# torchipeppo/prb-project-bearing-only-slam

Measured on AMD Instinct MI355X. Metric: GN iterations/sec + observations/sec (J+H build) at 1/2/4/8 GPUs vs CPU, higher is better.
Workload: dtype f32

## Files before the change

include/bos_host.h:

```cpp
#ifndef BOS_HOST_H_
#define BOS_HOST_H_

#include "bos.h"

#ifdef __cplusplus
extern "C" {
#endif

typedef struct bos_dataset bos_dataset;

int bos_dataset_load_g2o(const char* path, int triangulate, int verbose, bos_dataset** out);
int bos_dataset_synthetic(int32_t num_poses, int32_t num_landmarks, int32_t bearings_per_pose, uint64_t seed,
                          bos_dataset** out);
int bos_dataset_problem(const bos_dataset* ds, bos_problem* view);
const int32_t* bos_dataset_pose_ids(const bos_dataset* ds);
const int32_t* bos_dataset_landmark_ids(const bos_dataset* ds);
int32_t bos_dataset_fixed_pose_id(const bos_dataset* ds);
float bos_dataset_bound(const bos_dataset* ds);
int bos_dataset_ground_truth(const bos_dataset* ds, const double** pose_xyt, const double** landmark_xy);
int bos_dataset_write_g2o(const bos_dataset* ds, const char* path, const double* pose_xyt, const double* landmark_xy,
                          int with_landmarks);
void bos_dataset_free(bos_dataset* ds);

double bos_normalized_angle_f64(double a);
// ... 93 lines not shown

int bos_time_linearize(struct bos_solver* s, int32_t n, int32_t flush_caches, double* ms_per_build);
int bos_time_triangulate(struct bos_solver* s, int32_t n, double* ms_per_call);
int bos_time_steps(struct bos_solver* s, int32_t n, double* ms_per_step);

int bos_marginals_timing(const struct bos_solver* s, double ms[4], int64_t* sigma_bytes);
int bos_edge_covariances_timing(const struct bos_solver* s, double ms[5], int64_t* edge_bytes);
int bos_pair_covariances_timing(const struct bos_solver* s, double ms[6], int64_t* bytes);
int bos_node_covariances_timing(const struct bos_solver* s, double ms[7], int64_t* bytes);
int bos_associate_bearings_timing(const struct bos_solver* s, double ms[8], int64_t* bytes);
int bos_debug_set_associate_chunk(struct bos_solver* s, int64_t max_bearings);
int bos_match_timing(const struct bos_solver* s, double ms[8], int64_t* bytes);
int bos_debug_set_match_chunk(struct bos_solver* s, int64_t max_rows);
int bos_debug_set_pair_batch(struct bos_solver* s, int64_t max_distinct_nodes);
int bos_time_cost(struct bos_solver* s, int32_t n, double* ms_per_pass);

int bos_time_facade_steps(const bos_problem* problem, const bos_options* options, int32_t n, double* ms_per_step,
                          double* ms_state_read, double* ms_per_step_capi, int64_t* mismatches);
int bos_debug_facade_selftest(const bos_problem* problem, const bos_options* options, int32_t n, int64_t* mismatches);

void bos_debug_set_g2o_parser(int32_t line_by_line);
int bos_debug_inject_stall(struct bos_solver* s);
int bos_debug_set_step_graph(struct bos_solver* s, int32_t enable);
int bos_debug_solver_stamps(struct bos_solver* s, int64_t capacity, uint64_t* stamps, int32_t* meta);

enum {
    BOS_ROUTE_NONE = -1,
    BOS_ROUTE_F_REG16 = 0,
    BOS_ROUTE_F_REG16_SIDE = 1,
    BOS_ROUTE_F_PAN48 = 2,
    BOS_ROUTE_F_PAN64 = 3,
    BOS_ROUTE_F_PAN64_SIDE = 4,
    BOS_ROUTE_F_BLK = 5,
    BOS_ROUTE_F_BLK_SIDE2 = 6,
    BOS_ROUTE_F_MIXB_BLK = 7,
    BOS_ROUTE_F_MIXB_WAVE = 8,
    BOS_ROUTE_F_LEVEL = 9,
    BOS_ROUTE_F_FLOW = 10,
    BOS_ROUTE_F_FOLDED = 11,
    BOS_ROUTE_F_COUNT = 12
};
enum {
    BOS_ROUTE_B_FLOW = 0,
    BOS_ROUTE_B_WAVE = 1,
    BOS_ROUTE_B_LEVEL = 2,
    BOS_ROUTE_B_FOLD = 3,
// ... 22 lines not shown
```

prb-project-bearing-only-slam_amd/bos.py:

```python
from __future__ import annotations

import ctypes
import os
from typing import Optional

import numpy as np

_HERE = os.path.dirname(os.path.abspath(__file__))
LIB_PATH = os.path.join(_HERE, "lib", "libbos.so")
ALLOW_MISSING_SYMBOLS = False

BOS_OK = 0
BOS_FP64 = 64
BOS_FP32 = 32
BOS_SOLVER_SUPERNODAL = 0
BOS_SOLVER_DENSE_CHOL = 1
BOS_SOLVER_ROCSOLVER_RF = 2
BOS_SOLVER_SCHUR = 3
BOS_SOLVER_SPARSE_CHOL = BOS_SOLVER_SCHUR
BOS_PARTITION_SUBTREE = 0
BOS_PARTITION_OBSERVATIONS = 1
ABI_VERSION = 3

EXPORTED_SYMBOLS = [
    "bos_default_options", "bos_last_error", "bos_abi_version", "bos_device_count", "bos_device_peer_access",
    "bos_nccl_unique_id",
    "bos_create", "bos_destroy", "bos_set_kernel_threshold", "bos_set_damping_factor", "bos_step", "bos_step_n",
    "bos_linearize", "bos_linearize_async", "bos_synchronize", "bos_system_info_get", "bos_export_system",
    "bos_get_state", "bos_set_state", "bos_get_last_dx",
    "bos_dataset_load_g2o", "bos_dataset_synthetic", "bos_dataset_problem", "bos_dataset_pose_ids",
    "bos_dataset_landmark_ids", "bos_dataset_fixed_pose_id", "bos_dataset_bound", "bos_dataset_ground_truth",
    "bos_dataset_write_g2o", "bos_dataset_free", "bos_plan_inspect", "bos_plan_mf_selftest",
    "bos_debug_linearize_timeline", "bos_triangulate", "bos_triangulate_async", "bos_plan_shard_selftest",
    "bos_plan_node_owner", "bos_step_phase", "bos_exchange_size", "bos_exchange_download", "bos_exchange_upload",
    "bos_node_owner",
    "bos_debug_set_g2o_parser", "bos_debug_inject_stall", "bos_debug_set_step_graph", "bos_debug_solver_stamps",
    "bos_debug_solver_routes", "bos_debug_selinv_fronts", "bos_plan_mf_fronts",
    "bos_time_linearize", "bos_time_triangulate", "bos_time_steps", "bos_cpu_gn_create", "bos_cpu_gn_step", "bos_cpu_gn_get_state",
    "bos_cpu_gn_destroy", "bos_normalized_angle_f64", "bos_normalized_angle_f32", "bos_exchange_p2p_handle",
    "bos_exchange_p2p_connect", "bos_time_facade_steps", "bos_debug_facade_selftest", "bos_set_exchange_timeout",
    "bos_last_step_stamps", "bos_marginals", "bos_plan_mf_marginals", "bos_marginals_timing",
    "bos_lm_default_options", "bos_cost", "bos_optimize", "bos_time_cost", "bos_cpu_gn_set_kernel_threshold",
    "bos_cpu_gn_cost", "bos_cpu_gn_optimize", "bos_lm_rule_apply",
    "bos_edge_covariances", "bos_plan_mf_edge_covariances", "bos_edge_covariances_timing",
    "bos_pair_covariances", "bos_plan_mf_pair_covariances", "bos_plan_pair_paths", "bos_pair_covariances_timing",
    "bos_debug_set_pair_batch",
    "bos_node_covariances", "bos_plan_mf_node_covariances", "bos_node_covariances_timing",
    "bos_associate_bearings", "bos_plan_mf_associate_bearings", "bos_associate_bearings_timing",
    "bos_debug_set_associate_chunk", "bos_associate_tile",
    "bos_match_landmarks", "bos_match_poses", "bos_plan_mf_match_landmarks", "bos_plan_mf_match_poses",
    "bos_match_information_inverse", "bos_match_timing", "bos_debug_set_match_chunk",
]

LM_STOP_DX, LM_STOP_COST, LM_STOP_ITERATIONS, LM_STOP_LAMBDA = 1, 2, 3, 4
LM_MAX_ITERATIONS = 4096

P2P_HANDLE_BYTES = 64

_dp = ctypes.POINTER(ctypes.c_double)
_ip = ctypes.POINTER(ctypes.c_int32)
# ... 173 lines not shown
        "bos_cost": (ctypes.c_int, [vp, _dp, _dp, _ip]),
        "bos_optimize": (ctypes.c_int, [vp, ctypes.POINTER(bos_lm_options), ctypes.POINTER(bos_lm_result),
                                        ctypes.POINTER(bos_lm_iteration), ctypes.c_int32]),
        "bos_time_cost": (ctypes.c_int, [vp, ctypes.c_int32, _dp]),
        "bos_cpu_gn_set_kernel_threshold": (ctypes.c_int, [vp, ctypes.c_double]),
        "bos_cpu_gn_cost": (ctypes.c_int, [vp, _dp, _dp, _ip]),
        "bos_cpu_gn_optimize": (ctypes.c_int, [vp, ctypes.POINTER(bos_lm_options), ctypes.POINTER(bos_lm_result),
                                               ctypes.POINTER(bos_lm_iteration), ctypes.c_int32]),
        "bos_lm_rule_apply": (ctypes.c_int, [ctypes.POINTER(bos_lm_state), ctypes.POINTER(bos_lm_options), ctypes.c_double,
                                             ctypes.c_double, ctypes.c_double, ctypes.c_int32,
                                             ctypes.POINTER(bos_lm_iteration)]),
        "bos_plan_shard_selftest": (ctypes.c_int, [ctypes.POINTER(bos_problem), ctypes.POINTER(bos_options), ctypes.c_int32,
                                                   _dp, _dp, _dp]),
        "bos_plan_node_owner": (ctypes.c_int, [ctypes.POINTER(bos_problem), ctypes.POINTER(bos_options), ctypes.c_int32, _ip]),
        "bos_step_phase": (ctypes.c_int, [vp, ctypes.c_int32, ctypes.POINTER(bos_step_stats)]),
        "bos_exchange_size": (ctypes.c_int, [vp, ctypes.c_int32, ctypes.POINTER(ctypes.c_int64)]),
        "bos_exchange_download": (ctypes.c_int, [vp, ctypes.c_int32, _dp]),
        "bos_exchange_upload": (ctypes.c_int, [vp, ctypes.c_int32, _dp]),
        "bos_node_owner": (ctypes.c_int, [vp, _ip]),
        "bos_debug_set_g2o_parser": (None, [ctypes.c_int32]),
        "bos_debug_inject_stall": (ctypes.c_int, [vp]),
        "bos_debug_set_step_graph": (ctypes.c_int, [vp, ctypes.c_int32]),
        "bos_debug_solver_routes": (ctypes.c_int, [vp, ctypes.c_int64, _ip, _ip]),
        "bos_debug_selinv_fronts": (ctypes.c_int, [vp, ctypes.c_int64, _ip, _ip, _ip, _ip]),
        "bos_plan_mf_fronts": (ctypes.c_int, [ctypes.POINTER(bos_problem), ctypes.POINTER(bos_options), ctypes.c_int64, _ip, _ip]),
        "bos_debug_solver_stamps": (ctypes.c_int, [vp, ctypes.c_int64, ctypes.POINTER(ctypes.c_uint64),
                                                   ctypes.POINTER(ctypes.c_int32)]),
        "bos_time_linearize": (ctypes.c_int, [vp, ctypes.c_int32, ctypes.c_int32, _dp]),
        "bos_time_triangulate": (ctypes.c_int, [vp, ctypes.c_int32, _dp]),
        "bos_time_steps": (ctypes.c_int, [vp, ctypes.c_int32, _dp]),
        "bos_cpu_gn_create": (ctypes.c_int, [ctypes.POINTER(bos_problem), ctypes.c_int32, ctypes.c_int32,
                                             ctypes.POINTER(vp)]),
        "bos_cpu_gn_step": (ctypes.c_int, [vp, _dp]),
        "bos_cpu_gn_get_state": (ctypes.c_int, [vp, _dp, _dp]),
        "bos_cpu_gn_destroy": (None, [vp]),
        "bos_exchange_p2p_handle": (ctypes.c_int, [vp, ctypes.c_void_p]),
        "bos_exchange_p2p_connect": (ctypes.c_int, [vp, ctypes.c_void_p]),
        "bos_set_exchange_timeout": (ctypes.c_int, [vp, ctypes.c_double]),
        "bos_last_step_stamps": (ctypes.c_int, [vp, ctypes.POINTER(ctypes.c_uint64)]),
        "bos_normalized_angle_f64": (ctypes.c_double, [ctypes.c_double]),
        "bos_normalized_angle_f32": (ctypes.c_float, [ctypes.c_float]),
        "bos_time_facade_steps": (ctypes.c_int, [ctypes.POINTER(bos_problem), ctypes.POINTER(bos_options), ctypes.c_int32,
                                                 _dp, _dp, _dp, ctypes.POINTER(ctypes.c_int64)]),
        "bos_debug_facade_selftest": (ctypes.c_int, [ctypes.POINTER(bos_problem), ctypes.POINTER(bos_options),
                                                     ctypes.c_int32, ctypes.POINTER(ctypes.c_int64)]),
    }
# ... 409 lines not shown
    a, b, _ = _pair_cov_arrays(node_a, node_b, False, False, False)
    out = np.zeros((len(a), len(PAIR_PATH_COLS)), dtype=np.int32)
    opt = options(solver, schur_leaf=schur_leaf)
    _check(lib().bos_plan_pair_paths(ctypes.byref(cs), ctypes.byref(opt), len(a), _ptr(a, ctypes.c_int32),
                                     _ptr(b, ctypes.c_int32), _ptr(out, ctypes.c_int32)), "plan_pair_paths")
    return out


PLAN_FRONT_COLS = ("k", "r", "level", "parent", "children", "folded_children", "folded", "diag_records", "cross_rj",
                   "cross_jj", "cross_transposed")


def plan_mf_fronts(P: Problem, solver: int = BOS_SOLVER_SCHUR, schur_leaf: int = 0) -> np.ndarray:
    cs = P.c_struct()
    opt = options(solver, schur_leaf=schur_leaf)
    n = ctypes.c_int32(0)
    _check(lib().bos_plan_mf_fronts(ctypes.byref(cs), ctypes.byref(opt), 0, None, ctypes.byref(n)), "plan_mf_fronts")
    out = np.zeros((n.value, len(PLAN_FRONT_COLS)), dtype=np.int32)
    _check(lib().bos_plan_mf_fronts(ctypes.byref(cs), ctypes.byref(opt), out.size, _ptr(out, ctypes.c_int32),
                                    ctypes.byref(n)), "plan_mf_fronts")
    return out


def plan_shard_selftest(P: Problem, world: int, vals, rhs, solver: int = BOS_SOLVER_SCHUR):
    cs = P.c_struct()
    v = np.ascontiguousarray(vals, dtype=np.float64)
    b = np.ascontiguousarray(rhs, dtype=np.float64)
    x = np.zeros_like(b)
    opt = options(solver)
    _check(lib().bos_plan_shard_selftest(ctypes.byref(cs), ctypes.byref(opt), world, _ptr(v, ctypes.c_double),
                                         _ptr(b, ctypes.c_double), _ptr(x, ctypes.c_double)), "plan_shard_selftest")
    return x


def plan_node_owner(P: Problem, world: int, solver: int = BOS_SOLVER_SCHUR) -> np.ndarray:
    cs = P.c_struct()
    o = np.zeros(P.NP + P.NL, dtype=np.int32)
    opt = options(solver)
    _check(lib().bos_plan_node_owner(ctypes.byref(cs), ctypes.byref(opt), world, _ptr(o, ctypes.c_int32)),
           "plan_node_owner")
    return o


def lm_options(**opts) -> bos_lm_options:
    o = bos_lm_options()
    lib().bos_lm_default_options(ctypes.byref(o))
# ... 222 lines not shown
        out = np.zeros((n.value, 4), dtype=np.int32)
        _check(lib().bos_debug_solver_routes(self._h, out.size, _ptr(out, ctypes.c_int32), ctypes.byref(n)),
               "bos_debug_solver_routes")
        return out

    SELINV_CLASSES = ("wave_lds", "blk_lds_mfma", "blk_workspace")
    SELINV_COLS = ("class", "launch", "k", "r", "folded", "sigma_front", "diag_records", "cross_rj", "cross_jj",
                   "cross_transposed")

    def debug_selinv_fronts(self) -> dict:
        n = ctypes.c_int32(0)
        _check(lib().bos_debug_selinv_fronts(self._h, 0, None, ctypes.byref(n), None, None), "bos_debug_selinv_fronts")
        fronts = np.zeros((n.value, len(self.SELINV_COLS)), dtype=np.int32)
        node = np.zeros(self.P.NP + self.P.NL, dtype=np.int32)
        edge = np.zeros(len(self.P.b_z) + len(self.P.o_z), dtype=np.int32)
        _check(lib().bos_debug_selinv_fronts(self._h, fronts.size, _ptr(fronts, ctypes.c_int32), ctypes.byref(n),
                                             _ptr(node, ctypes.c_int32), _ptr(edge, ctypes.c_int32)),
               "bos_debug_selinv_fronts")
        return {"fronts": fronts, "node_front": node, "edge_front": edge}

    def debug_set_step_graph(self, enable: bool):
        _check(lib().bos_debug_set_step_graph(self._h, int(enable)), "bos_debug_set_step_graph")

    def time_linearize(self, n: int, flush_caches: bool = False) -> float:
        ms = ctypes.c_double(0)
        _check(lib().bos_time_linearize(self._h, n, int(flush_caches), ctypes.byref(ms)), "bos_time_linearize")
        return ms.value

    def time_steps(self, n: int) -> float:
        ms = ctypes.c_double(0)
        _check(lib().bos_time_steps(self._h, n, ctypes.byref(ms)), "bos_time_steps")
        return ms.value

    def time_triangulate(self, n: int) -> float:
        ms = ctypes.c_double(0)
        _check(lib().bos_time_triangulate(self._h, n, ctypes.byref(ms)), "bos_time_triangulate")
        return ms.value

    def triangulate(self):
        _check(lib().bos_triangulate(self._h), "bos_triangulate")

    def triangulate_async(self):
        _check(lib().bos_triangulate_async(self._h), "bos_triangulate_async")

    def synchronize(self):
        _check(lib().bos_synchronize(self._h), "bos_synchronize")
# ... 163 lines not shown
```

prb-project-bearing-only-slam_amd/csrc/hip/mf_backward.hpp:

```cpp
#pragma once

#include <hip/hip_runtime.h>

#include <cstdint>

#include "mf_device.hpp"
#include "mf_flow.hpp"
#include "wave_util.hpp"

namespace bos {
namespace dev {

namespace {

constexpr int kBwdRegK = 32;

template <int MODE>
__device__ __forceinline__ void backward_front(const MfArgs& a, int s, double* w, int lane, const Flow* f,
                                               const int32_t* parent) {
    constexpr bool COH = MODE == kModeFlow;
    const int k = a.k[s], r = a.r[s], m = k + r;
    const int c0 = a.col0[s];
    const int32_t* fi = a.findex + a.findex_off[s];
    double* t = w + k;
// ... 147 lines not shown
    }
    if (head) {
        const double x1 = (y1 - t1) / L11;
        t0 += L10 * x1;
        a.x[c0] = (y0 - t0) / L00;
        a.x[c0 + 1] = x1;
    }
}

__global__ __launch_bounds__(64) void mf_backward_flow(const MfArgs a, const Flow f_in, const int32_t* parent) {
    extern __shared__ __attribute__((aligned(16))) double w[];
    Flow f = f_in;
    f.epoch = *f_in.epoch_src;
    for (int it = 0; it <= f.n; ++it) {
        const int t = next_ticket(f.ticket);
        if (t >= f.n) break;
        const int s = f.order[t];
        backward_front<kModeFlow>(a, s, w, threadIdx.x, &f, parent);
        fstamp(f.stamps, s, 4);
    }
    leave_flow(f);
}

}

}
}
```

prb-project-bearing-only-slam_amd/csrc/hip/multifrontal.hip:

```cpp
#include <hip/hip_runtime.h>

#include <algorithm>
#include <cstdint>
#include <string>
#include <vector>

#include "../../../include/bos_host.h"
#include "../host/plan.hpp"
#include "device_mem.hpp"
#include "mf_backward.hpp"
#include "mf_blk.hpp"
#include "mf_device.hpp"
#include "mf_flow.hpp"
#include "mf_level.hpp"
#include "mf_wave.hpp"
#include "multifrontal.hpp"
#include "selinv.hpp"

namespace bos {
namespace dev {

constexpr int kClasses = 6;
inline int front_class(int m) { return m <= kMfWaveMaxM ? (m - 1) / 16 : m <= kBlkMaxM ? 4 : 5; }
inline int launch_class(int m) {
    const int c = front_class(m);
    return c == 1 ? 2 : c;
}

struct Prog {
    int id = 0;
// ... 47 lines not shown
    hipStream_t side = nullptr, side2 = nullptr;
    hipEvent_t ev_fork = nullptr, ev_join = nullptr, ev_join2 = nullptr;
    static constexpr int tiny16 = 256;
    Prog prog[2];
    int8_t *fid_f = nullptr, *fid_b = nullptr;
    int32_t* parent = nullptr;
    int* tickets = nullptr;
    uint32_t* epoch = nullptr;
    unsigned long long* stamps = nullptr;
    int32_t *fold_cnt = nullptr, *fold_cptr = nullptr, *fold_chunk = nullptr, *fold_rec = nullptr;
    int16_t* emap = nullptr;
    int64_t* emap_off = nullptr;
    int32_t *col0 = nullptr, *k = nullptr, *r = nullptr, *child_ptr = nullptr, *child = nullptr,
            *rmap = nullptr, *amap_ptr = nullptr, *amap_src = nullptr, *amap_dst = nullptr, *findex = nullptr,
            *info = nullptr;
    int64_t *L_off = nullptr, *U_off = nullptr, *u_off = nullptr, *scratch_off = nullptr, *rmap_off = nullptr,
            *findex_off = nullptr;
    double *L = nullptr, *U = nullptr, *u = nullptr, *scratch = nullptr;
    const float* A32 = nullptr;
    int64_t pl_lo = 0;
    unsigned long long *Ug = nullptr, *xg = nullptr;
    int64_t* ug_off = nullptr;
    int8_t* xtag = nullptr;
    SelInv* selinv = nullptr;
    std::vector<int8_t> route_f, route_b;
    std::vector<int32_t> h_child_ptr, h_child, h_fold_cnt;
    bool noted_f[2] = {false, false}, noted_b[2] = {false, false};
    void note_f(int which, int route, const int32_t* fronts, int n) {
        if (noted_f[which]) return;
        for (int i = 0; i < n; ++i) {
            const int s = fronts[i];
            route_f[s] = (int8_t)route;
            if (!h_fold_cnt.empty())
                for (int ci = h_child_ptr[s]; ci < h_child_ptr[s] + h_fold_cnt[s]; ++ci)
                    route_f[h_child[ci]] = (int8_t)BOS_ROUTE_F_FOLDED;
        }
    }
    void note_b(int which, int route, const int32_t* fronts, int n) {
        if (noted_b[which]) return;
        for (int i = 0; i < n; ++i) route_b[fronts[i]] = (int8_t)route;
    }

    MfArgs args(const Prog& P, int lev, int c, const double* A, double* x) const {
        MfArgs g;
        g.level = P.list + (P.ptr.empty() ? 0 : P.ptr[lev * kClasses + c]);
        g.count = P.ptr.empty() ? 0 : P.count(lev, c);
// ... 165 lines not shown
    auto up = [&](auto** p, const auto& v) { return mem.upload(p, v, kMfPad); };
    auto bad = [&] { err = "device allocation or upload failed (multifrontal)"; return -2; };
    if (!(up(&d->fid_f, fid_f) && up(&d->fid_b, fid_b) && up(&d->parent, F.parent))) return bad();
    {
        std::vector<int64_t> ugo(F.nsuper, -1);
        int64_t ug_size = 0, ndof = 0;
        for (int c = 0; c < F.nsuper; ++c) {
            ndof = std::max<int64_t>(ndof, (int64_t)F.col0[c] + F.k[c]);
            const int p = F.parent[c];
            if (p < 0 || fid_f[c] == 0 || fid_f[p] != fid_f[c]) continue;
            const int64_t rc2 = F.r[c];
            ugo[c] = ug_size;
            ug_size += 2 * (rc2 * (rc2 + 1) / 2 + rc2);
        }
        std::vector<int8_t> xt(F.nsuper, 0);
        for (int c = 0; c < F.nsuper; ++c)
            if (fid_b[c] != 0)
                for (int q = c; q >= 0 && !xt[q]; q = F.parent[q]) xt[q] = 1;
        if (!(up(&d->ug_off, ugo) && up(&d->xtag, xt) && mem.alloc(&d->Ug, std::max<int64_t>(ug_size, 1), true, 2 * kMfPad) &&
              mem.alloc(&d->xg, std::max<int64_t>(2 * ndof, 1), true, 2 * kMfPad)))
            return bad();
    }
    if (!(mem.alloc(&d->tickets, 2 * kMfTickets, true) && mem.upload(&d->epoch, std::vector<uint32_t>{1}))) return bad();
    {
        std::vector<int64_t> eoff(F.nsuper, 0);
        std::vector<int16_t> em;
        for (int c = 0; c < F.nsuper; ++c) {
            const int p = F.parent[c];
            if (p < 0) continue;
            const int mp = F.k[p] + F.r[p], rc = F.r[c];
            if (mp > kBlkMaxM || rc == 0) continue;
            bool folded = false;
            for (int ci = F.child_ptr[p]; ci < F.child_ptr[p] + (F.fold_cnt.empty() ? 0 : F.fold_cnt[p]); ++ci)
                folded = folded || F.child[ci] == c;
            if (folded) continue;
            eoff[c] = (int64_t)em.size();
            const int32_t* rm = F.rmap.data() + F.rmap_off[c];
            for (int j = 0; j < rc; ++j)
                for (int i = j; i < rc; ++i) {
                    const int I = rm[i], J = rm[j];
                    if (I < J || I >= mp) { err = "multifrontal: child row map not increasing"; return -1; }
                    em.push_back((int16_t)(mp <= kMfWaveMaxM ? J * mp - J * (J - 1) / 2 + (I - J) : I + J * mp));
                }
        }
        if (!(up(&d->emap, em) && up(&d->emap_off, eoff))) return bad();
    }
// ... 110 lines not shown
                     d->fid_f, P.id, d->stamps};
        const int grid = std::min(P.n_flow_factor, d->ncu * kFlowWavesFactor);
        hipLaunchKernelGGL((mf_factor_flow<F32>), dim3(grid), dim3(64), 0, s, d->args(P, 0, 0, A, x), f);
        d->note_f(which, BOS_ROUTE_F_FLOW, P.h_order_factor.data(), P.n_flow_factor);
        if ((e = hipGetLastError()) != hipSuccess) return e;
    }
    d->noted_f[which] = true;
    return hipSuccess;
}

hipError_t mf_factor(MfDevice* d, int which, const double* A, double* x, hipStream_t s) {
    return d->A32 ? mf_factor_t<true>(d, which, A, x, s) : mf_factor_t<false>(d, which, A, x, s);
}

void mf_set_fold_source(MfDevice* d, const float* A32, int64_t pl_lo) {
    d->A32 = A32;
    d->pl_lo = pl_lo;
}

hipError_t mf_solve(MfDevice* d, int which, double* x, hipStream_t s) {
    hipError_t e;
    const Prog& P = d->prog[which];
    if (P.ptr.empty()) return hipSuccess;
    if (P.flow_solve) {
        const Flow fb{P.order_bwd, P.n_flow_solve, d->tickets + 1, d->tickets + kMfTickets + 1,
                      d->epoch, 0u, d->fid_b, P.id, d->stamps ? d->stamps + 8 * (int64_t)d->nsuper : nullptr};
        const int grid = std::min(P.n_flow_solve, d->ncu * kFlowWavesBackward);
        hipLaunchKernelGGL(mf_backward_flow, dim3(grid), dim3(64), P.lds_bwd_flow, s, d->args(P, 0, 0, nullptr, x), fb,
                           (const int32_t*)d->parent);
        d->note_b(which, BOS_ROUTE_B_FLOW, P.h_order_bwd.data(), P.n_flow_solve);
        if ((e = hipGetLastError()) != hipSuccess) return e;
    }
    for (int l = std::min(P.solve_lev0, d->nlevels) - 1; l >= 0; --l) {
        int n;
        if (P.bptr[l + 1] > P.bptr[l]) {
            MfArgs g = d->args(P, l, 0, nullptr, x);
            g.level = P.blist + P.bptr[l];
            g.count = P.bptr[l + 1] - P.bptr[l];
            hipLaunchKernelGGL(mf_backward_wave, dim3(g.count), dim3(64), P.blds[l], s, g);
            d->note_b(which, BOS_ROUTE_B_WAVE, P.h_blist.data() + P.bptr[l], g.count);
        }
        if ((n = P.count(l, 4, kClasses))) {
            MfArgs g = d->args(P, l, 4, nullptr, x);
            g.count = n;
            hipLaunchKernelGGL(mf_backward_level, dim3(n), dim3(kMfBlock), P.lds_max(P.lds_bwd, l, 4, kClasses), s, g);
            d->note_b(which, BOS_ROUTE_B_LEVEL, P.hl(l, 4), n);
        }
        if ((e = hipGetLastError()) != hipSuccess) return e;
    }
    if (P.n_fold > 0) {
        MfArgs g = d->args(P, 0, 0, nullptr, x);
        g.level = P.fold_list;
        g.count = P.n_fold;
        hipLaunchKernelGGL(mf_backward_fold, dim3(((int64_t)P.n_fold * kFoldLanes + kMfBlock - 1) / kMfBlock), dim3(kMfBlock), 0, s, g);
        d->note_b(which, BOS_ROUTE_B_FOLD, P.h_fold_list.data(), P.n_fold);
        if ((e = hipGetLastError()) != hipSuccess) return e;
    }
    d->noted_b[which] = true;
    return hipSuccess;
}

int mf_debug_routes(const MfDevice* d, int8_t* factor, int8_t* backward) {
    for (int w = 0; w < 2; ++w)
        if (!d->prog[w].ptr.empty() && (!d->noted_f[w] || !d->noted_b[w])) return -1;
    std::copy(d->route_f.begin(), d->route_f.end(), factor);
    std::copy(d->route_b.begin(), d->route_b.end(), backward);
    return 0;
}

MfView mf_view(const MfDevice* d) { return MfView{d->k, d->r, d->parent, d->rmap, d->L_off, d->rmap_off, d->L}; }
SelInv** mf_selinv_slot(MfDevice* d) { return &d->selinv; }
int32_t* mf_info_ptr(const MfDevice* d) { return d->info; }
uint32_t* mf_epoch_ptr(const MfDevice* d) { return d->epoch; }
void mf_debug_set_stamps(MfDevice* d, unsigned long long* stamps) {
    d->stamps = stamps;
#ifdef BOS_MF_PIVOT_CYCLES
    unsigned long long* b = stamps ? stamps + 8 * (int64_t)d->nsuper : nullptr;
    (void)hipMemcpyToSymbol(HIP_SYMBOL(g_pivot_bwd), &b, sizeof(b));
#endif
}
int32_t* mf_tickets_ptr(const MfDevice* d) { return d->tickets; }
double* mf_update_ptr(const MfDevice* d) { return d->U; }
double* mf_uvec_ptr(const MfDevice* d) { return d->u; }

hipError_t mf_debug_skip_next_front(MfDevice* d, hipStream_t s) {
    if (d->prog[0].n_flow_factor == 0 || !d->prog[0].first_waited) return hipErrorInvalidValue;
    static const int one = 1;
    return hipMemcpyAsync(d->tickets, &one, sizeof(int), hipMemcpyHostToDevice, s);
}

// ... 3 lines not shown
```

prb-project-bearing-only-slam_amd/csrc/hip/multifrontal.hpp:

```cpp
#pragma once

#include <hip/hip_runtime.h>

#include <string>

namespace bos {
struct Multifrontal;
namespace dev {

struct MfDevice;

int mf_create(const Multifrontal& F, const int8_t* owner, int rank, MfDevice** out, std::string& err);
void mf_destroy(MfDevice* d);
hipError_t mf_factor(MfDevice* d, int program, const double* A, double* x, hipStream_t s);
void mf_set_fold_source(MfDevice* d, const float* A32, int64_t pl_lo);
hipError_t mf_solve(MfDevice* d, int program, double* x, hipStream_t s);
double* mf_update_ptr(const MfDevice* d);
double* mf_uvec_ptr(const MfDevice* d);
int32_t* mf_info_ptr(const MfDevice* d);
uint32_t* mf_epoch_ptr(const MfDevice* d);
void mf_debug_set_stamps(MfDevice* d, unsigned long long* stamps);
constexpr int32_t kMfStall = 1 << 30;
int mf_debug_routes(const MfDevice* d, int8_t* factor, int8_t* backward);
int32_t* mf_tickets_ptr(const MfDevice* d);
constexpr int kMfTickets = 3;
struct MfView {
    const int32_t *k, *r, *parent, *rmap;
    const int64_t *L_off, *rmap_off;
    const double* L;
};
MfView mf_view(const MfDevice* d);
struct SelInv;
SelInv** mf_selinv_slot(MfDevice* d);
hipError_t mf_debug_skip_next_front(MfDevice* d, hipStream_t s);

}
}
```

prb-project-bearing-only-slam_amd/csrc/hip/solver_step.hip:

```cpp
#include <algorithm>
#include <atomic>
#include <chrono>
#include <cstring>

#include "solver_handle.hpp"

using namespace bos::capi;

namespace {

template <typename T> bos::dev::LinParams<T> lin_params(const bos_solver* s) {
    bos::dev::LinParams<T> p;
    p.pc = (const T*)s->d_pc;
    p.pth = (const T*)s->d_pth;
    p.lc = (const T*)s->d_lc;
    const bos::Plan& P = s->plan;
    p.NP = s->NP;
    p.lane_pose = s->lane_identity ? nullptr : s->lane_pose;
    p.n_groups = (int)P.blk.lane_pose.size();
    p.n_lm_lanes = (int)P.blk.lm_lane_lm.size();
    p.pose_blocks = s->pose_blocks;
    p.pose_b0 = (int)s->pose_b0;
    p.n_pose_run = (int)s->n_pose_run;
    p.lm_b0 = (int)s->lm_b0;
// ... 574 lines not shown
    const bos::Multifrontal& F = s->plan.mf;
    if (nsuper) *nsuper = F.nsuper;
    if (!routes && capacity == 0 && nsuper) return BOS_OK;
    if (!routes || capacity < 4 * (int64_t)F.nsuper) return fail(BOS_ERR_INVALID, "routes: capacity 4 * supernodes");
    std::vector<int8_t> rf(F.nsuper), rb(F.nsuper);
    if (bos::dev::mf_debug_routes(s->mf, rf.data(), rb.data()))
        return fail(BOS_ERR_INVALID, "routes: no step has been enqueued on this handle yet");
    for (int x = 0; x < F.nsuper; ++x) {
        routes[4 * x] = rf[x];
        routes[4 * x + 1] = rb[x];
        routes[4 * x + 2] = F.k[x];
        routes[4 * x + 3] = F.r[x];
    }
    return BOS_OK;
}

int bos_debug_set_step_graph(bos_solver* s, int32_t enable) {
    if (!s) return fail(BOS_ERR_INVALID, "null handle");
    drop_graph(s);
    s->graph_failed = !enable;
    return BOS_OK;
}

int bos_triangulate(bos_solver* s) {
    if (!s) return fail(BOS_ERR_INVALID, "null handle");
    HIP_TRY(hipSetDevice(s->device));
    int rc = enqueue_triangulate(s);
    if (rc) return rc;
    HIP_TRY(hipStreamSynchronize(s->stream));
    s->have_dx = false;
    return BOS_OK;
}

int bos_triangulate_async(bos_solver* s) {
    if (!s) return fail(BOS_ERR_INVALID, "null handle");
    return enqueue_triangulate(s);
}

int bos_synchronize(bos_solver* s) {
    if (!s) return fail(BOS_ERR_INVALID, "null handle");
    HIP_TRY(hipStreamSynchronize(s->stream));
    return BOS_OK;
}

int bos_linearize(bos_solver* s, bos_step_stats* st) {
    if (!s) return fail(BOS_ERR_INVALID, "null handle");
// ... 141 lines not shown
```

prb-project-bearing-only-slam_amd/csrc/host/capi_host.cpp:

```cpp
#include <chrono>
#include <cstdio>
#include <cstdlib>
#include <algorithm>
#include <cmath>
#include <cstring>
#include <functional>
#include <memory>
#include <stdexcept>
#include <string>
#include <vector>

#include "../../../include/bos_host.h"
#include "associate.hpp"
#include "match.hpp"
#include "edge_cov.hpp"
#include "node_cov.hpp"
#include "pair_cov.hpp"
#include "g2o_utils.hpp"
#include "host_mf.hpp"
#include "plan.hpp"
#include "synthetic.hpp"
#include "triangulation.hpp"

#include "error.hpp"

namespace {
int hfail(int code, const std::string& m) { return bos::set_error(code, m); }
}

struct bos_dataset {
    proj02::State state;
    proj02::BearingObservationVector bearings;
    proj02::OdometryObservationVector odometry;
    int fixed_pose_id = -1;
    float bound = 0;
    std::vector<double> pose_xyt, lm_xy, b_z, o_z, o_om;
// ... 341 lines not shown
    for (int32_t x : F.fold_list) folded[x] = 1;
    std::vector<int32_t> out_ptr, out_rec;
    bos::CrossRecords cr;
    if (!bos::selinv_records(P, out_ptr, out_rec) ||
        !bos::selinv_cross_records(P, pi.Mb, pi.Mo, pi.b_pose, pi.b_lm, pi.o_src, pi.o_dst, cr))
        return hfail(BOS_ERR_UNSUPPORTED, "a node or an edge's cross block is not inside one front");
    for (int x = 0; x < F.nsuper; ++x) {
        int32_t* o = fronts + (size_t)BOS_PLAN_FRONT_COLS * x;
        o[0] = F.k[x]; o[1] = F.r[x]; o[2] = lev[x]; o[3] = F.parent[x];
        o[4] = F.child_ptr[x + 1] - F.child_ptr[x];
        o[5] = F.fold_cnt.empty() ? 0 : F.fold_cnt[x];
        o[6] = folded[x];
        o[7] = out_ptr[x + 1] - out_ptr[x];
        o[8] = o[9] = o[10] = 0;
        for (int q = cr.ptr[x]; q < cr.ptr[x + 1]; ++q) {
            const int32_t* rec = cr.rec.data() + (size_t)bos::kCrossRec * q;
            ++o[rec[0] >= F.k[x] ? 8 : 9];
            o[10] += rec[5];
        }
    }
    return BOS_OK;
}

int bos_plan_mf_selftest(const bos_problem* pb, const bos_options* options, const double* vals, const double* rhs,
                         double* x) {
    if (!pb || !vals || !rhs || !x) return hfail(BOS_ERR_INVALID, "null argument");
    bos::ProblemIndex pi;
    bos_options opt;
    int fmode = 0;
    int rc = plan_args(pb, options, pi, fmode, opt);
    if (rc) return rc;
    if (opt.solver != BOS_SOLVER_SUPERNODAL && opt.solver != BOS_SOLVER_SCHUR)
        return hfail(BOS_ERR_INVALID, "selftest needs a multifrontal solver");
    bos::Plan P;
    std::string err;
    rc = bos::build_plan(pi, 0, 1, fmode, P, err);
    if (rc) return hfail(rc, err);
    bos::HostMf M(P, vals, rhs);
    auto all = [](int) { return true; };
    M.factor(all);
    M.forward(all);
    M.backward(all);
    std::copy(M.x.begin(), M.x.end(), x);
    return BOS_OK;
}

// ... 523 lines not shown
```

Measured before the change: 87.86 billion.

## Solve top supernodal levels with one wave per root-to-leaf path

Adds a backward-solve route where each base-level front gets a single wave that walks its chain of ancestors to the root. Each wave redundantly recomputes the shared upper fronts in its own LDS copy of the solution, and it prefetches the next front's panel into registers while solving the current one. This replaces the per-level launches or ticket-based flow solve for the upper levels and so removes inter-front synchronisation and launch overhead. The cost is redundant work on shared ancestors, an extra kernel that saves the right-hand side first, and a limit on LDS and front size. The route is on by default when the plan qualifies, and it falls back when occupancy is insufficient.

```diff
diff --git a/include/bos_host.h b/include/bos_host.h
--- a/include/bos_host.h
+++ b/include/bos_host.h
@@ -139,6 +139,10 @@
 void bos_debug_set_g2o_parser(int32_t line_by_line);
 int bos_debug_inject_stall(struct bos_solver* s);
 int bos_debug_set_step_graph(struct bos_solver* s, int32_t enable);
+int bos_debug_set_backward_path(struct bos_solver* s, int32_t enable);
+int bos_debug_backward_path_info(struct bos_solver* s, int32_t* out);
+int bos_plan_backward_path(const bos_problem* problem, const bos_options* options, int32_t world, int32_t* info,
+                           int32_t* fronts, int32_t* base, int32_t* path_ptr, int32_t* path, int32_t* rows);
 int bos_debug_solver_stamps(struct bos_solver* s, int64_t capacity, uint64_t* stamps, int32_t* meta);
 
 enum {
diff --git a/prb-project-bearing-only-slam_amd/bos.py b/prb-project-bearing-only-slam_amd/bos.py
--- a/prb-project-bearing-only-slam_amd/bos.py
+++ b/prb-project-bearing-only-slam_amd/bos.py
@@ -36,6 +36,7 @@
     "bos_node_owner",
     "bos_debug_set_g2o_parser", "bos_debug_inject_stall", "bos_debug_set_step_graph", "bos_debug_solver_stamps",
     "bos_debug_solver_routes", "bos_debug_selinv_fronts", "bos_plan_mf_fronts",
+    "bos_debug_set_backward_path", "bos_debug_backward_path_info", "bos_plan_backward_path",
     "bos_time_linearize", "bos_time_triangulate", "bos_time_steps", "bos_cpu_gn_create", "bos_cpu_gn_step", "bos_cpu_gn_get_state",
     "bos_cpu_gn_destroy", "bos_normalized_angle_f64", "bos_normalized_angle_f32", "bos_exchange_p2p_handle",
     "bos_exchange_p2p_connect", "bos_time_facade_steps", "bos_debug_facade_selftest", "bos_set_exchange_timeout",
@@ -255,6 +256,10 @@
         "bos_debug_inject_stall": (ctypes.c_int, [vp]),
         "bos_debug_set_step_graph": (ctypes.c_int, [vp, ctypes.c_int32]),
         "bos_debug_solver_routes": (ctypes.c_int, [vp, ctypes.c_int64, _ip, _ip]),
+        "bos_debug_set_backward_path": (ctypes.c_int, [vp, ctypes.c_int32]),
+        "bos_debug_backward_path_info": (ctypes.c_int, [vp, _ip]),
+        "bos_plan_backward_path": (ctypes.c_int, [ctypes.POINTER(bos_problem), ctypes.POINTER(bos_options), ctypes.c_int32,
+                                                  _ip, _ip, _ip, _ip, _ip, _ip]),
         "bos_debug_selinv_fronts": (ctypes.c_int, [vp, ctypes.c_int64, _ip, _ip, _ip, _ip]),
         "bos_plan_mf_fronts": (ctypes.c_int, [ctypes.POINTER(bos_problem), ctypes.POINTER(bos_options), ctypes.c_int64, _ip, _ip]),
         "bos_debug_solver_stamps": (ctypes.c_int, [vp, ctypes.c_int64, ctypes.POINTER(ctypes.c_uint64),
@@ -710,6 +715,24 @@
     return out
 
 
+def plan_backward_path(P: Problem, solver: int = BOS_SOLVER_SCHUR, schur_leaf: int = 0, world: int = 1) -> dict:
+    cs = P.c_struct()
+    opt = options(solver, schur_leaf=schur_leaf)
+    info = np.zeros(8, dtype=np.int32)
+    ip = lambda a: _ptr(a, ctypes.c_int32)
+    _check(lib().bos_plan_backward_path(ctypes.byref(cs), ctypes.byref(opt), world, ip(info), None, None, None, None, None),
+           "plan_backward_path")
+    fronts = np.zeros((info[4], 7), dtype=np.int32)
+    base = np.zeros(max(info[1], 1), dtype=np.int32)
+    path_ptr = np.zeros(info[1] + 1, dtype=np.int32)
+    path = np.zeros(max(info[5], 1), dtype=np.int32)
+    rows = np.zeros((max(info[6], 1), 2), dtype=np.int32)
+    _check(lib().bos_plan_backward_path(ctypes.byref(cs), ctypes.byref(opt), world, ip(info), ip(fronts), ip(base),
+                                        ip(path_ptr), ip(path), ip(rows)), "plan_backward_path")
+    return {"base_level": int(info[0]), "base_fronts": int(info[1]), "longest_path": int(info[2]), "lds_bytes": int(info[3]),
+            "fronts": fronts, "base": base[:info[1]], "path_ptr": path_ptr, "path": path[:info[5]], "rows": rows[:info[6]]}
+
+
 def plan_shard_selftest(P: Problem, world: int, vals, rhs, solver: int = BOS_SOLVER_SCHUR):
     cs = P.c_struct()
     v = np.ascontiguousarray(vals, dtype=np.float64)
@@ -978,6 +1001,14 @@
     def debug_set_step_graph(self, enable: bool):
         _check(lib().bos_debug_set_step_graph(self._h, int(enable)), "bos_debug_set_step_graph")
 
+    def debug_set_backward_path(self, enable: bool):
+        _check(lib().bos_debug_set_backward_path(self._h, int(enable)), "bos_debug_set_backward_path")
+
+    def backward_path_info(self) -> dict:
+        out = np.zeros(4, dtype=np.int32)
+        _check(lib().bos_debug_backward_path_info(self._h, _ptr(out, ctypes.c_int32)), "bos_debug_backward_path_info")
+        return dict(zip(("base_level", "base_fronts", "longest_path", "lds_bytes"), (int(v) for v in out)))
+
     def time_linearize(self, n: int, flush_caches: bool = False) -> float:
         ms = ctypes.c_double(0)
         _check(lib().bos_time_linearize(self._h, n, int(flush_caches), ctypes.byref(ms)), "bos_time_linearize")
diff --git a/prb-project-bearing-only-slam_amd/csrc/hip/mf_backward.hpp b/prb-project-bearing-only-slam_amd/csrc/hip/mf_backward.hpp
--- a/prb-project-bearing-only-slam_amd/csrc/hip/mf_backward.hpp
+++ b/prb-project-bearing-only-slam_amd/csrc/hip/mf_backward.hpp
@@ -193,7 +193,145 @@
     leave_flow(f);
 }
 
-}
-
-}
-}
+struct PathArgs {
+    const int32_t *k, *r, *col0;
+    const int64_t *L_off, *findex_off;
+    const double* L;
+    double* x;
+    unsigned long long* stamps;
+    const int32_t* path_ptr;
+    const int32_t* path;
+    const int32_t* pbase;
+    const int32_t* rowpos;
+    const int32_t* stamper;
+    const double* y;
+    int nx;
+};
+
+__global__ __launch_bounds__(256) void mf_path_save_y(const int32_t* dof, int n, const double* x, double* y) {
+    const int i = blockIdx.x * 256 + threadIdx.x;
+    if (i < n) y[dof[i]] = x[dof[i]];
+}
+
+constexpr int kPathPre = 8;
+struct PathMeta {
+    int k, r, c0, pb;
+    int64_t L_off, fi_off;
+};
+struct PathPre {
+    double v[kPathPre], y;
+    int pos;
+};
+
+__device__ __forceinline__ int64_t readlane_i64(int64_t x, int l) {
+    const int lo = __builtin_amdgcn_readlane((int)(x & 0xffffffffll), l);
+    const int hi = __builtin_amdgcn_readlane((int)(x >> 32), l);
+    return ((int64_t)hi << 32) | (unsigned int)lo;
+}
+
+__device__ __forceinline__ PathMeta path_meta(const PathMeta& mine, int i) {
+    PathMeta f;
+    f.k = __builtin_amdgcn_readlane(mine.k, i);
+    f.r = __builtin_amdgcn_readlane(mine.r, i);
+    f.c0 = __builtin_amdgcn_readlane(mine.c0, i);
+    f.pb = __builtin_amdgcn_readlane(mine.pb, i);
+    f.L_off = readlane_i64(mine.L_off, i);
+    f.fi_off = readlane_i64(mine.fi_off, i);
+    return f;
+}
+
+__device__ __forceinline__ void path_prefetch(const PathArgs& p, const PathMeta& f, int lane, PathPre& o) {
+    const double* src = p.L + f.L_off;
+    const int n = (f.k + f.r) * f.k;
+#pragma unroll
+    for (int u = 0; u < kPathPre; ++u) o.v[u] = src[min(64 * u + lane, n - 1)];
+    o.y = p.y[f.c0 + min(lane, f.k - 1)];
+    o.pos = p.rowpos[f.fi_off + f.k + min(lane, max(f.r - 1, 0))];
+}
+
+template <int KR>
+__device__ __forceinline__ double path_chain_reg(const double* Lw, int k, int m, int lane, bool own, int col, double yv,
+                                                 double tj, double rjj) {
+    double lr[KR], xv = 0.0;
+#pragma unroll
+    for (int j = 0; j < KR; ++j) lr[j] = own && j < k ? Lw[j + col * m] : 0.0;
+#pragma unroll
+    for (int j = KR - 1; j >= 0; --j) {
+        if (j < k) {
+            const double xj = readlane_d((yv - tj) * rjj, j);
+            if (lane == j) xv = xj;
+            else if (lane < j) tj += lr[j] * xj;
+        }
+    }
+    return xv;
+}
+
+__global__ __launch_bounds__(64) void mf_backward_path(const PathArgs p) {
+    extern __shared__ __attribute__((aligned(16))) double w[];
+    double* const xp = w;
+    double* const Lw = w + p.nx;
+    const int lane = threadIdx.x, b = blockIdx.x;
+    const int p0 = p.path_ptr[b], n = p.path_ptr[b + 1] - p0;
+    PathMeta mine;
+    {
+        const int s = p.path[p0 + min(lane, n - 1)];
+        mine.k = p.k[s];
+        mine.r = p.r[s];
+        mine.c0 = p.col0[s];
+        mine.pb = p.pbase[s];
+        mine.L_off = p.L_off[s];
+        mine.fi_off = p.findex_off[s];
+    }
+    PathMeta f = path_meta(mine, 0);
+    PathPre pre;
+    path_prefetch(p, f, lane, pre);
+    for (int i = 0; i < n; ++i) {
+        const int k = f.k, r = f.r, m = k + r, c0 = f.c0, pb = f.pb;
+        int s = 0;
+        unsigned long long* stp = nullptr;
+        if (p.stamps) {
+            s = p.path[p0 + i];
+            stp = p.stamper[s] == b ? p.stamps : nullptr;
+        }
+        fstamp(stp, s, 0);
+#pragma unroll
+        for (int u = 0; u < kPathPre; ++u)
+            if (64 * u + lane < m * k) Lw[64 * u + lane] = pre.v[u];
+        if (m * k > 64 * kPathPre)
+            stage_lds<8, false>(Lw + 64 * kPathPre, p.L + f.L_off + 64 * kPathPre, m * k - 64 * kPathPre, lane);
+        const bool own = lane < k;
+        const int col = own ? lane : 0;
+        const double yv = own ? pre.y : 0.0;
+        const double xr = xp[lane < r ? pre.pos : 0];
+        wave_sync();
+        fstamp(stp, s, 1);
+        fstamp(stp, s, 2);
+        f = path_meta(mine, min(i + 1, n - 1));
+        path_prefetch(p, f, lane, pre);
+        const double rjj = own ? 1.0 / Lw[col + col * m] : 1.0;
+        double tj = 0.0;
+        for (int q = 0; q < r; ++q) tj += Lw[k + q + col * m] * readlane_d(xr, q);
+        double xv = 0.0;
+        if (k <= 16) xv = path_chain_reg<16>(Lw, k, m, lane, own, col, yv, tj, rjj);
+        else if (k <= kBwdRegK) xv = path_chain_reg<kBwdRegK>(Lw, k, m, lane, own, col, yv, tj, rjj);
+        else {
+            for (int j = k - 1; j >= 0; --j) {
+                const double xj = readlane_d((yv - tj) * rjj, j);
+                if (lane == j) xv = xj;
+                else if (lane < j) tj += Lw[j + col * m] * xj;
+            }
+        }
+        if (own) {
+            xp[pb + lane] = xv;
+            p.x[c0 + lane] = xv;
+        }
+        wave_sync();
+        fstamp(stp, s, 3);
+        fstamp(stp, s, 4);
+    }
+}
+
+}
+
+}
+}
diff --git a/prb-project-bearing-only-slam_amd/csrc/hip/multifrontal.hip b/prb-project-bearing-only-slam_amd/csrc/hip/multifrontal.hip
--- a/prb-project-bearing-only-slam_amd/csrc/hip/multifrontal.hip
+++ b/prb-project-bearing-only-slam_amd/csrc/hip/multifrontal.hip
@@ -6,6 +6,7 @@
 #include <vector>
 
 #include "../../../include/bos_host.h"
+#include "../host/backward_path.hpp"
 #include "../host/plan.hpp"
 #include "device_mem.hpp"
 #include "mf_backward.hpp"
@@ -99,6 +100,12 @@
     unsigned long long *Ug = nullptr, *xg = nullptr;
     int64_t* ug_off = nullptr;
     int8_t* xtag = nullptr;
+    BackwardPath bp;
+    bool path_on = true;
+    int32_t *bp_path_ptr = nullptr, *bp_path = nullptr, *bp_pbase = nullptr, *bp_rowpos = nullptr, *bp_stamper = nullptr,
+            *bp_ydof = nullptr;
+    double* bp_y = nullptr;
+    std::vector<int32_t> h_path_fronts;
     SelInv* selinv = nullptr;
     std::vector<int8_t> route_f, route_b;
     std::vector<int32_t> h_child_ptr, h_child, h_fold_cnt;
@@ -310,6 +317,30 @@
             return bad();
     }
     if (!(mem.alloc(&d->tickets, 2 * kMfTickets, true) && mem.upload(&d->epoch, std::vector<uint32_t>{1}))) return bad();
+    if (!owner) {
+        BackwardPath& bp = d->bp;
+        build_backward_path(F, bp);
+        int resident = 0;
+        if (bp.on() &&
+            (hipOccupancyMaxActiveBlocksPerMultiprocessor(&resident, mf_backward_path, 64, bp.lds_bytes) != hipSuccess ||
+             (int64_t)resident * d->ncu < (int64_t)bp.base.size())) {
+            (void)hipGetLastError();
+            bp = BackwardPath();
+        }
+        if (bp.on()) {
+            std::vector<int32_t> stamper(F.nsuper, -1);
+            for (size_t b = 0; b < bp.base.size(); ++b)
+                for (int q = bp.path_ptr[b]; q < bp.path_ptr[b + 1]; ++q)
+                    if (stamper[bp.path[q]] < 0) stamper[bp.path[q]] = (int32_t)b;
+            d->h_path_fronts.assign(F.level.begin() + F.level_ptr[bp.base_level], F.level.begin() + F.level_ptr[F.nlevels]);
+            int64_t ndof = 0;
+            for (int c = 0; c < F.nsuper; ++c) ndof = std::max<int64_t>(ndof, (int64_t)F.col0[c] + F.k[c]);
+            if (!(up(&d->bp_path_ptr, bp.path_ptr) && up(&d->bp_path, bp.path) && up(&d->bp_pbase, bp.pbase) &&
+                  up(&d->bp_rowpos, bp.rowpos) && up(&d->bp_stamper, stamper) && up(&d->bp_ydof, bp.ydof) &&
+                  mem.alloc(&d->bp_y, std::max<int64_t>(ndof, 1), true, kMfPad)))
+                return bad();
+        }
+    }
     {
         std::vector<int64_t> eoff(F.nsuper, 0);
         std::vector<int16_t> em;
@@ -466,7 +497,19 @@
     hipError_t e;
     const Prog& P = d->prog[which];
     if (P.ptr.empty()) return hipSuccess;
-    if (P.flow_solve) {
+    const bool path = which == 0 && d->path_on && d->bp.on();
+    if (path) {
+        const BackwardPath& bp = d->bp;
+        const int ny = (int)bp.ydof.size();
+        hipLaunchKernelGGL(mf_path_save_y, dim3((ny + 255) / 256), dim3(256), 0, s, (const int32_t*)d->bp_ydof, ny,
+                           (const double*)x, d->bp_y);
+        const PathArgs pa{d->k, d->r, d->col0, d->L_off, d->findex_off, d->L, x,
+                          d->stamps ? d->stamps + 8 * (int64_t)d->nsuper : nullptr,
+                          d->bp_path_ptr, d->bp_path, d->bp_pbase, d->bp_rowpos, d->bp_stamper, d->bp_y, bp.nx};
+        hipLaunchKernelGGL(mf_backward_path, dim3((int)bp.base.size()), dim3(64), bp.lds_bytes, s, pa);
+        d->note_b(which, BOS_ROUTE_B_FLOW, d->h_path_fronts.data(), (int)d->h_path_fronts.size());
+        if ((e = hipGetLastError()) != hipSuccess) return e;
+    } else if (P.flow_solve) {
         const Flow fb{P.order_bwd, P.n_flow_solve, d->tickets + 1, d->tickets + kMfTickets + 1,
                       d->epoch, 0u, d->fid_b, P.id, d->stamps ? d->stamps + 8 * (int64_t)d->nsuper : nullptr};
         const int grid = std::min(P.n_flow_solve, d->ncu * kFlowWavesBackward);
@@ -475,7 +518,7 @@
         d->note_b(which, BOS_ROUTE_B_FLOW, P.h_order_bwd.data(), P.n_flow_solve);
         if ((e = hipGetLastError()) != hipSuccess) return e;
     }
-    for (int l = std::min(P.solve_lev0, d->nlevels) - 1; l >= 0; --l) {
+    for (int l = (path ? d->bp.base_level : std::min(P.solve_lev0, d->nlevels)) - 1; l >= 0; --l) {
         int n;
         if (P.bptr[l + 1] > P.bptr[l]) {
             MfArgs g = d->args(P, l, 0, nullptr, x);
@@ -510,6 +553,18 @@
     std::copy(d->route_f.begin(), d->route_f.end(), factor);
     std::copy(d->route_b.begin(), d->route_b.end(), backward);
     return 0;
+}
+
+void mf_debug_set_backward_path(MfDevice* d, bool on) {
+    d->path_on = on;
+    d->noted_b[0] = false;
+}
+void mf_backward_path_info(const MfDevice* d, int32_t out[4]) {
+    const bool on = d->path_on && d->bp.on();
+    out[0] = on ? d->bp.base_level : 0;
+    out[1] = on ? (int32_t)d->bp.base.size() : 0;
+    out[2] = on ? d->bp.longest : 0;
+    out[3] = on ? d->bp.lds_bytes : 0;
 }
 
 MfView mf_view(const MfDevice* d) { return MfView{d->k, d->r, d->parent, d->rmap, d->L_off, d->rmap_off, d->L}; }
diff --git a/prb-project-bearing-only-slam_amd/csrc/hip/multifrontal.hpp b/prb-project-bearing-only-slam_amd/csrc/hip/multifrontal.hpp
--- a/prb-project-bearing-only-slam_amd/csrc/hip/multifrontal.hpp
+++ b/prb-project-bearing-only-slam_amd/csrc/hip/multifrontal.hpp
@@ -22,6 +22,8 @@
 void mf_debug_set_stamps(MfDevice* d, unsigned long long* stamps);
 constexpr int32_t kMfStall = 1 << 30;
 int mf_debug_routes(const MfDevice* d, int8_t* factor, int8_t* backward);
+void mf_debug_set_backward_path(MfDevice* d, bool on);
+void mf_backward_path_info(const MfDevice* d, int32_t out[4]);
 int32_t* mf_tickets_ptr(const MfDevice* d);
 constexpr int kMfTickets = 3;
 struct MfView {
diff --git a/prb-project-bearing-only-slam_amd/csrc/hip/solver_step.hip b/prb-project-bearing-only-slam_amd/csrc/hip/solver_step.hip
--- a/prb-project-bearing-only-slam_amd/csrc/hip/solver_step.hip
+++ b/prb-project-bearing-only-slam_amd/csrc/hip/solver_step.hip
@@ -620,6 +620,21 @@
     return BOS_OK;
 }
 
+int bos_debug_set_backward_path(bos_solver* s, int32_t enable) {
+    if (!s) return fail(BOS_ERR_INVALID, "null handle");
+    if (!uses_mf(s)) return fail(BOS_ERR_UNSUPPORTED, "multifrontal handles only");
+    drop_graph(s);
+    bos::dev::mf_debug_set_backward_path(s->mf, enable != 0);
+    return BOS_OK;
+}
+
+int bos_debug_backward_path_info(bos_solver* s, int32_t* out) {
+    if (!s || !out) return fail(BOS_ERR_INVALID, "null argument");
+    if (!uses_mf(s)) return fail(BOS_ERR_UNSUPPORTED, "multifrontal handles only");
+    bos::dev::mf_backward_path_info(s->mf, out);
+    return BOS_OK;
+}
+
 int bos_triangulate(bos_solver* s) {
     if (!s) return fail(BOS_ERR_INVALID, "null handle");
     HIP_TRY(hipSetDevice(s->device));
diff --git a/prb-project-bearing-only-slam_amd/csrc/host/backward_path.hpp b/prb-project-bearing-only-slam_amd/csrc/host/backward_path.hpp
--- /dev/null
+++ b/prb-project-bearing-only-slam_amd/csrc/host/backward_path.hpp
@@ -0,0 +1,109 @@
+#pragma once
+
+#include <algorithm>
+#include <cstdint>
+#include <vector>
+
+#include "plan.hpp"
+
+namespace bos {
+
+constexpr int kPathMaxM = 64;
+constexpr int kPathCus = 256, kPathWavesPerCu = 8;
+constexpr int kPathLdsPerCu = 160 * 1024, kPathLdsMax = 48 * 1024;
+#ifndef BOS_MF_PATH_BASE_MIN
+#define BOS_MF_PATH_BASE_MIN 2
+#endif
+constexpr int kPathBaseMin = BOS_MF_PATH_BASE_MIN;
+
+struct BackwardPath {
+    int base_level = 0;
+    int longest = 0;
+    int panel = 0, nx = 0;
+    int lds_bytes = 0;
+    std::vector<int32_t> base;
+    std::vector<int32_t> path_ptr;
+    std::vector<int32_t> path;
+    std::vector<int32_t> pbase;
+    std::vector<int32_t> rowpos;
+    std::vector<int32_t> ydof;
+    bool on() const { return !base.empty(); }
+};
+
+inline void build_backward_path(const Multifrontal& F, BackwardPath& P) {
+    P = BackwardPath();
+    const int L = F.nlevels;
+    std::vector<int32_t> lev(F.nsuper, -1);
+    for (int l = 0; l < L; ++l)
+        for (int q = F.level_ptr[l]; q < F.level_ptr[l + 1]; ++q) lev[F.level[q]] = l;
+    const int B0 = std::max(std::min(kPathBaseMin, L), std::min(2, L));
+    for (int q = F.level_ptr[B0]; q < F.level_ptr[L]; ++q)
+        if (F.k[F.level[q]] + F.r[F.level[q]] > kPathMaxM) return;
+    std::vector<int32_t> pbase(F.nsuper, -1), depth(F.nsuper, 0);
+    for (int B = B0; B < L; ++B) {
+        int panel = 0, nx = 0, longest = 0;
+        bool ok = true;
+        for (int l = L - 1; l >= B && ok; --l)
+            for (int q = F.level_ptr[l]; q < F.level_ptr[l + 1] && ok; ++q) {
+                const int s = F.level[q], p = F.parent[s];
+                ok = p < 0 || lev[p] > l;
+                if (!ok) break;
+                pbase[s] = p < 0 ? 0 : pbase[p] + F.k[p];
+                depth[s] = p < 0 ? 1 : depth[p] + 1;
+                panel = std::max(panel, (F.k[s] + F.r[s]) * F.k[s]);
+                nx = std::max(nx, pbase[s] + F.k[s]);
+                longest = std::max(longest, depth[s]);
+            }
+        const int n = F.level_ptr[B + 1] - F.level_ptr[B];
+        const int lds = (nx + panel) * 8;
+        if (!ok || longest > 64 || lds > kPathLdsMax) return;
+        if (n > kPathCus * std::min(kPathWavesPerCu, kPathLdsPerCu / std::max(lds, 1))) continue;
+        std::vector<int8_t> seen(F.nsuper, 0);
+        std::vector<int32_t> path_ptr{0}, path, chain;
+        for (int q = F.level_ptr[B]; q < F.level_ptr[B + 1]; ++q) {
+            chain.clear();
+            for (int s = F.level[q]; s >= 0; s = F.parent[s]) chain.push_back(s);
+            for (auto it = chain.rbegin(); it != chain.rend(); ++it) {
+                path.push_back(*it);
+                seen[*it] = 1;
+            }
+            path_ptr.push_back((int32_t)path.size());
+        }
+        bool covered = true;
+        for (int q = F.level_ptr[B]; q < F.level_ptr[L] && covered; ++q) covered = seen[F.level[q]] != 0;
+        if (!covered) return;
+        std::vector<int32_t> rowpos(F.findex.size(), -1);
+        for (int q = F.level_ptr[B]; q < F.level_ptr[L] && covered; ++q) {
+            const int s = F.level[q], k = F.k[s], m = k + F.r[s];
+            const int32_t* fi = F.findex.data() + F.findex_off[s];
+            for (int i = 0; i < k && covered; ++i) {
+                covered = fi[i] == F.col0[s] + i;
+                rowpos[F.findex_off[s] + i] = pbase[s] + i;
+            }
+            int a = F.parent[s];
+            for (int i = k; i < m && covered; ++i) {
+                while (a >= 0 && !(fi[i] >= F.col0[a] && fi[i] < F.col0[a] + F.k[a])) a = F.parent[a];
+                covered = a >= 0;
+                if (covered) rowpos[F.findex_off[s] + i] = pbase[a] + (fi[i] - F.col0[a]);
+            }
+        }
+        if (!covered) return;
+        P.base_level = B;
+        P.longest = longest;
+        P.panel = panel;
+        P.nx = nx;
+        P.lds_bytes = lds;
+        P.base.assign(F.level.begin() + F.level_ptr[B], F.level.begin() + F.level_ptr[B + 1]);
+        P.path_ptr = std::move(path_ptr);
+        P.path = std::move(path);
+        for (int s = 0; s < F.nsuper; ++s)
+            if (lev[s] < B) pbase[s] = -1;
+        P.pbase = pbase;
+        P.rowpos = std::move(rowpos);
+        for (int q = F.level_ptr[B]; q < F.level_ptr[L]; ++q)
+            for (int j = 0; j < F.k[F.level[q]]; ++j) P.ydof.push_back(F.col0[F.level[q]] + j);
+        return;
+    }
+}
+
+}
diff --git a/prb-project-bearing-only-slam_amd/csrc/host/capi_host.cpp b/prb-project-bearing-only-slam_amd/csrc/host/capi_host.cpp
--- a/prb-project-bearing-only-slam_amd/csrc/host/capi_host.cpp
+++ b/prb-project-bearing-only-slam_amd/csrc/host/capi_host.cpp
@@ -12,6 +12,7 @@
 
 #include "../../../include/bos_host.h"
 #include "associate.hpp"
+#include "backward_path.hpp"
 #include "match.hpp"
 #include "edge_cov.hpp"
 #include "node_cov.hpp"
@@ -399,6 +400,48 @@
     return BOS_OK;
 }
 
+int bos_plan_backward_path(const bos_problem* pb, const bos_options* options, int32_t world, int32_t* info, int32_t* fronts,
+                           int32_t* base, int32_t* path_ptr, int32_t* path, int32_t* rows) {
+    if (!pb || !info || world < 1) return hfail(BOS_ERR_INVALID, "bad argument");
+    bos::ProblemIndex pi;
+    bos_options opt;
+    int fmode = 0;
+    int rc = plan_args(pb, options, pi, fmode, opt);
+    if (rc) return rc;
+    if (opt.solver != BOS_SOLVER_SUPERNODAL && opt.solver != BOS_SOLVER_SCHUR)
+        return hfail(BOS_ERR_INVALID, "the backward path needs a multifrontal solver");
+    bos::Plan P;
+    std::string err;
+    rc = bos::build_plan(pi, 0, world, fmode, P, err);
+    if (rc) return hfail(rc, err);
+    const bos::Multifrontal& F = P.mf;
+    bos::BackwardPath bp;
+    bos::build_backward_path(F, bp);
+    if (F.findex.size() > (size_t)INT32_MAX) return hfail(BOS_ERR_UNSUPPORTED, "front index beyond int32");
+    info[0] = bp.base_level; info[1] = (int32_t)bp.base.size(); info[2] = bp.longest; info[3] = bp.lds_bytes;
+    info[4] = F.nsuper; info[5] = (int32_t)bp.path.size(); info[6] = (int32_t)F.findex.size(); info[7] = 0;
+    if (fronts) {
+        std::vector<int32_t> lev(F.nsuper, -1);
+        for (int l = 0; l < F.nlevels; ++l)
+            for (int q = F.level_ptr[l]; q < F.level_ptr[l + 1]; ++q) lev[F.level[q]] = l;
+        for (int x = 0; x < F.nsuper; ++x) {
+            int32_t* o = fronts + 7 * (size_t)x;
+            o[0] = F.k[x]; o[1] = F.r[x]; o[2] = lev[x]; o[3] = F.parent[x]; o[4] = F.col0[x];
+            o[5] = bp.on() ? bp.pbase[x] : -1;
+            o[6] = (int32_t)F.findex_off[x];
+        }
+    }
+    if (base) std::copy(bp.base.begin(), bp.base.end(), base);
+    if (path_ptr && bp.on()) std::copy(bp.path_ptr.begin(), bp.path_ptr.end(), path_ptr);
+    if (path) std::copy(bp.path.begin(), bp.path.end(), path);
+    if (rows)
+        for (size_t e = 0; e < F.findex.size(); ++e) {
+            rows[2 * e] = F.findex[e];
+            rows[2 * e + 1] = bp.on() ? bp.rowpos[e] : -1;
+        }
+    return BOS_OK;
+}
+
 int bos_plan_mf_selftest(const bos_problem* pb, const bos_options* options, const double* vals, const double* rhs,
                          double* x) {
     if (!pb || !vals || !rhs || !x) return hfail(BOS_ERR_INVALID, "null argument");
```

Result: slower. 78.57 billion (-10.6%).
